# ZhonghuaYi/FocusFlow_official

Hardware: AMD Instinct MI355X
Metric: frame-pairs/sec FF-RAFT 384x512 iters=12 (higher is better)
Workload: dtype f32 via fp16x3 split operands on the f16 MFMA pipe (f32 accumulate, fp32-level accuracy); 1 GPU; FF-RAFT forward (test_mode), 8 pairs/GPU 384x512, iters=12, fp32 correlation pyramid, random-init weights, ORB-like masks (BASELINE configs[1]); pairs_per_gpu=8, corr_pyramid=fp32, conv_precision=f16x3, hipgraph=False, skip_unused_upsample=False, parallelism=dp1 (independent shards, no collective)

## Files before the change

### focusflow_official_amd/_hip.py

```python
import ctypes as C
import os

_PKG = os.path.dirname(os.path.abspath(__file__))
LIB_PATH = os.path.join(_PKG, "lib", "libfocusflow_hip.so")
if os.environ.get("FF_LAB_LIB"):
    LIB_PATH = os.path.join(_PKG, "lib", os.environ["FF_LAB_LIB"])

ACT_NONE, ACT_RELU, ACT_SIGMOID, ACT_TANH, ACT_LEAKY = 0, 1, 2, 3, 4
W_F32, W_F16X3, W_F16 = 0, 1, 2
MAX_SEG = 3
_fp = C.c_void_p
_ll = C.c_longlong


class FFFusionPair(C.Structure):
    _fields_ = [
        ("x", _fp * 2), ("x_ld", C.c_int * 2), ("xres", _fp * 2), ("xres_ld", C.c_int * 2), ("scale", _fp * 2), ("shift", _fp * 2),
        ("in_act", C.c_int), ("w_frag", _fp * 2), ("bias", _fp * 2), ("w_format", C.c_int), ("y", _fp * 2), ("y_ld", C.c_int * 2),
        ("B", C.c_int), ("HW", C.c_int), ("C", C.c_int),
    ]


class FFConvParams(C.Structure):
    _fields_ = [
# ... 17 lines not shown

PACK_MAX_MEMBERS = 4
PACK_MAX_SLICES = 4


class FFPackJob(C.Structure):
    _fields_ = [
        ("w", _fp * PACK_MAX_MEMBERS), ("bias", _fp * PACK_MAX_MEMBERS),
        ("cout_m", C.c_int * PACK_MAX_MEMBERS), ("off", C.c_int * PACK_MAX_MEMBERS), ("nmem", C.c_int), ("cout", C.c_int),
        ("cin_src", C.c_int), ("nslice", C.c_int), ("slice_lo", C.c_int * PACK_MAX_SLICES), ("slice_hi", C.c_int * PACK_MAX_SLICES),
        ("cin", C.c_int), ("cin_pad", C.c_int), ("KH", C.c_int), ("KW", C.c_int),
        ("fwd", _fp), ("bias_dst", _fp), ("dgrad", _fp),
        ("fwd_format", C.c_int), ("dgrad_format", C.c_int), ("cout_pad", C.c_int), ("reserved", C.c_int),
        ("items_fwd", _ll), ("items_dgrad", _ll), ("block0", _ll),
    ]


_SIGS = {
    "ff_pack_job_check": [C.POINTER(FFPackJob)],
    "ff_pack_weights_table": [_fp, C.c_int, _ll, _fp],
    "ff_unpack_wgrad_group": [_fp, _fp, C.c_int, C.POINTER(C.c_int), C.POINTER(C.c_int), C.POINTER(C.c_int), C.c_int, C.c_int,
                              C.POINTER(C.c_int), C.POINTER(C.c_int), C.c_int, C.c_int, C.c_int, _fp, _fp],
    "ff_conv2d_fwd": [C.POINTER(FFConvParams), _fp],
    "ff_pack_conv_weight": [_fp, C.c_int, C.c_int, C.c_int, C.c_int, _fp, C.c_int, C.c_int, _fp],
    "ff_pack_split_f16": [_fp, _fp, _ll, C.c_int, _fp],
    "ff_pack_frag16": [_fp, _fp, C.c_int, C.c_int, _fp],
    "ff_norm_stats": [_fp, C.c_int, C.c_int, C.c_int, C.c_int, C.c_int, _fp, _fp],
    "ff_norm_stats_finish": [_fp, C.c_int, C.c_int, C.c_int, _fp, _fp],
    "ff_mask_upsample_pack": [_fp, _fp, _fp],
    "ff_mask_upsample_fwd": [_fp, C.c_int, _fp, C.c_int, _fp, C.c_float, _fp, C.c_int, _fp, C.c_int, C.c_int, C.c_int, _fp],
    "ff_probe_memory_kernel": [_fp, _ll, _fp, _ll, C.c_int, C.c_int, C.c_int, C.c_uint, C.POINTER(C.c_longlong), C.POINTER(C.c_longlong), _fp],
    "ff_launch_timing_begin": [C.c_int],
    "ff_launch_timing_end": [C.c_int, C.POINTER(C.c_longlong), C.POINTER(C.c_double), C.POINTER(C.c_double), C.POINTER(C.c_double)],
    "ff_norm_apply": [_fp, C.c_int, _fp, C.c_int, C.c_int, C.c_int, C.c_int, _fp, C.c_int, C.c_float,
                      _fp, _fp, C.c_int, _fp, C.c_int, _fp],
    "ff_norm_coeffs": [_fp, C.c_int, C.c_int, _ll, C.c_float, _fp, _fp, _fp, _fp, _fp],
    "ff_bn_fold": [_fp, _fp, _fp, _fp, C.c_float, _fp, _fp, C.c_int, _fp],
    "ff_bn_update_running": [_fp, _ll, C.c_float, _fp, _fp, C.c_int, _fp],
    "ff_prep_input": [_fp, C.c_int, C.c_float, _fp, C.c_int, C.c_int, C.c_int, _fp],
    "ff_corr_pyramid": [_fp, _fp, _fp, _fp, _ll, C.c_int, C.c_int, _fp],
    "ff_corr_lookup_fwd": [C.POINTER(_fp), C.c_int, C.c_int, _fp, _ll, C.c_int, C.c_int, _fp, C.c_int, _fp, _fp],
    "ff_corr_build": [_fp, _fp, C.POINTER(_fp), C.c_int, C.c_int, C.c_int, C.c_int, C.c_int, _fp],
    "ff_corr_retile": [_fp, _fp, _ll, C.c_int, C.c_int, C.c_int, C.c_int, C.c_int, _fp],
    "ff_corr_tile_rows": [_fp, _fp, C.c_int, C.c_int, C.c_int, C.c_int, C.c_int, _fp],
    "ff_corr_lookup_tiled_fwd": [C.POINTER(_fp), C.c_int, _fp, _ll, C.c_int, C.c_int, _fp, C.c_int, _fp, _fp],
    "ff_corr_lookup_tiled_bwd_all": [_fp, C.POINTER(_fp), C.POINTER(_fp), C.c_int, C.c_int, _ll, C.c_int, C.c_int, _fp],
# ... 147 lines not shown
```

### focusflow_official_amd/csrc/conv_patch.hip

```cpp
#include <algorithm>
#include <cstdlib>
#include "ff_common.h"

namespace {

typedef float f32x16 __attribute__((ext_vector_type(16)));
typedef float f32x4 __attribute__((ext_vector_type(4)));
typedef _Float16 f16x8 __attribute__((ext_vector_type(8)));
typedef _Float16 f16x4 __attribute__((ext_vector_type(4)));

constexpr int TW = 16, ROWB = 128;
constexpr int ROWP = 144;
__device__ __forceinline__ int PI16(int i) { return (i >= 4 && i < 12) ? 2 * (i - 4) : (i < 4 ? 2 * i + 1 : 2 * (i - 12) + 9); }
__device__ __forceinline__ int KG16(int g) { return ((g & 1) << 1) | (g >> 1); }


struct PArgs {
    FFConvParams p;
    int Cin, nci;
    int tiles_x, tiles_y, n_tiles;
    long long w_row_bytes;
    int nci_split;
};

__device__ __forceinline__ void split4(const f32x4 v, f16x4& h0, f16x4& h1) {
#pragma unroll
    for (int j = 0; j < 4; ++j) {
        const _Float16 a = (_Float16)v[j];
        h0[j] = a;
        h1[j] = (_Float16)(v[j] - (float)a);
    }
}

template <int TERMS, int NITEM, int TM, int TN, int ABL, int WB, bool PIN = false, bool INORM = false, bool SPLITK = false, bool MF16 = false, int EPI = 0, bool STATS = false>
__device__ __forceinline__ void conv_patch_body(const PArgs& a) {
    constexpr int TH = 4 * TM, BN = 64 * TN, NW = 2 * TN;
    extern __shared__ __attribute__((aligned(16))) char smem[];
    const FFConvParams& p = a.p;
    float xs, xinv;
    ff::input_scale(p.x_amax, xs, xinv);
    xs *= ff::XSPLIT; xinv *= ff::SPLIT_INV;
    const int KH = p.KH, KW = p.KW, PH = TH + KH - 1, PW = TW + KW - 1, NPIX = PH * PW;
    char* sP = smem;
    char* sW = smem + ((NPIX * ROWP + 255) & ~255);

// ... 262 lines not shown

    const int li = lane & 31, lh = lane >> 5;
    const int rot = (KW - 1) & 15;
    const int lrow = li >> 4, lcol = ((li & 15) - lrow * rot) & 15;
    const int ntaps = KH * KW;
    const int brow = wn * TN * 32 + li;
    const char* abase[TM];
#pragma unroll
    for (int t = 0; t < TM; ++t) abase[t] = sP + (((wm * TM + t) * 2 + lrow) * PW + lcol) * ROWP + lh * 16;

    f16x8 abl_f;
#pragma unroll
    for (int i = 0; i < 8; ++i) abl_f[i] = (_Float16)(0.37f + 0.01f * (float)((lane * 7 + i * 3) & 31));
    const int c_beg = SPLITK ? (int)blockIdx.y * a.nci_split : 0;
    const int c_end = SPLITK ? min(c_beg + a.nci_split, a.nci) : a.nci;
    load_patch(c_beg);
    load_w(c_beg);
    int wbuf = 0;
    for (int c = c_beg; c < c_end; ++c) {
        __syncthreads();
        if (ABL != 6 || c == c_beg) store_patch();
        store_w(wbuf);
        __syncthreads();
        if (c + 1 < c_end && ABL != 6) load_patch(c + 1);
        for (int tap = 0; tap < ntaps; ++tap) {
            const bool last = tap + 1 == ntaps;
            const int next_kc = last ? (c + 1) : (tap + 1) * a.nci + c;
            if (!(last && c + 1 == c_end) && ABL != 1 && ABL != 2) load_w(last ? c + 1 : next_kc);
            if (PIN) __builtin_amdgcn_sched_barrier(0);
            const int dy = tap / KW, dx = tap - dy * KW;
            const int tapoff = (dy * PW + dx) * ROWP;
            const char* cW = sW + wbuf * BN * ROWP + brow * ROWP + lh * 16;
#pragma unroll
            for (int s = 0; s < 2; ++s) {
                f16x8 a0[TM], a1[TM], b0[TN], b1[TN];
                if constexpr (ABL == 5) {
#pragma unroll
                    for (int t = 0; t < TM; ++t) { a0[t] = abl_f; a1[t] = abl_f; }
#pragma unroll
                    for (int j = 0; j < TN; ++j) { b0[j] = abl_f; b1[j] = abl_f; }
                    asm volatile("" : "+v"(abl_f));
                } else {
#pragma unroll
                for (int t = 0; t < TM; ++t) {
                    const char* pa = abase[t] + tapoff;
                    a0[t] = *reinterpret_cast<const f16x8*>(pa + s * 32);
                    if (TERMS == 3) a1[t] = *reinterpret_cast<const f16x8*>(pa + 64 + s * 32);
// ... 3 lines not shown
                    b0[j] = *reinterpret_cast<const f16x8*>(cW + j * 32 * ROWP + s * 32);
                    if (TERMS == 3) b1[j] = *reinterpret_cast<const f16x8*>(cW + j * 32 * ROWP + 64 + s * 32);
                }
                }
#pragma unroll
                for (int t = 0; t < TM; ++t)
#pragma unroll
                    for (int j = 0; j < TN; ++j) {
                        if constexpr (ABL == 3) {
                            asm volatile("" :: "v"(a0[t]), "v"(b0[j]));
                            if (TERMS == 3) asm volatile("" :: "v"(a1[t]), "v"(b1[j]));
                            continue;
                        }
                        acc[t][j] = __builtin_amdgcn_mfma_f32_32x32x16_f16(a0[t], b0[j], acc[t][j], 0, 0, 0);
                        if (TERMS == 3) {
                            acc[t][j] = __builtin_amdgcn_mfma_f32_32x32x16_f16(a0[t], b1[j], acc[t][j], 0, 0, 0);
                            acc[t][j] = __builtin_amdgcn_mfma_f32_32x32x16_f16(a1[t], b0[j], acc[t][j], 0, 0, 0);
                        }
                    }
            }
            if (!last && ABL != 2) {
                if (WB == 1 && ABL != 4) __syncthreads();
                store_w(WB == 1 ? 0 : wbuf ^ 1);
                if (ABL != 4) __syncthreads();
                if (WB == 2) wbuf ^= 1;
            }
        }
        if (WB == 2) wbuf ^= 1;
    }

    if constexpr (SPLITK) {
        float* ws = p.splitk_ws + (long long)blockIdx.y * pix_total * p.Cout;
#pragma unroll
        for (int j = 0; j < TN; ++j) {
            const int n = n0 + (wn * TN + j) * 32 + li;
            if (n >= p.Cout) continue;
#pragma unroll
            for (int t = 0; t < TM; ++t)
#pragma unroll
                for (int r = 0; r < 16; ++r) {
                    const int pi = (r & 3) + 8 * (r >> 2) + 4 * lh;
                    const int y = y0 + (wm * TM + t) * 2 + (pi >> 4), x = x0 + ((pi - (pi >> 4) * rot) & 15);
                    if (y < H && x < W) ws[(((long long)bimg * H + y) * W + x) * p.Cout + n] = acc[t][j][r] * xinv;
                }
        }
        return;
// ... 77 lines not shown
}

template <int TERMS, int NITEM, int TM, int TN, int ABL = 0, int WB = 2>
__global__ __launch_bounds__(256) void conv_patch_kernel(const PArgs a) { conv_patch_body<TERMS, NITEM, TM, TN, ABL, WB>(a); }
template <int TERMS, int NITEM, int TM, int TN, int OCC, bool PIN = true, int ABL = 0, bool INORM = false, bool SPLITK = false, bool MF16 = false, int EPI = 0, bool STATS = false>
__global__ __launch_bounds__(256) __attribute__((amdgpu_waves_per_eu(OCC, OCC))) void conv_patch_kernel_occ(const PArgs a) { conv_patch_body<TERMS, NITEM, TM, TN, ABL, 1, PIN, INORM, SPLITK, MF16, EPI, STATS>(a); }

__global__ __launch_bounds__(256) void splitk_finish_kernel(const FFConvParams p, int splits, long long npix) {
    const long long total = npix * p.Cout;
    for (long long i = blockIdx.x * 256ll + threadIdx.x; i < total; i += (long long)gridDim.x * 256) {
        const long long m = i / p.Cout;
        const int n = (int)(i - m * p.Cout);
        float v = 0.f;
        for (int s = 0; s < splits; ++s) v += p.splitk_ws[(long long)s * total + i];
        v += p.bias ? p.bias[n] : 0.f;
        v *= p.out_scale;
        if (p.ch_scale) v = v * p.ch_scale[n] + p.ch_shift[n];
        v = ff::apply_act(v, p.act);
        if (p.res) v = ff::apply_act(v + p.res[m * p.res_ld + n], p.act_res);
        p.y[m * p.y_ld + n] = v;
    }
}

template <int TERMS, int NITEM, int TM, int TN, int OCC>
int launch_occ(const PArgs& a, size_t lds, hipStream_t s) {
    const long long blocks = (long long)a.p.B * a.tiles_y * a.tiles_x * a.n_tiles;
    static const bool mf16 = ff::tune_env("FF_MFMA16") && atoi(ff::tune_env("FF_MFMA16")) == 1;
    if (a.p.stats_part) {
        if (a.p.in_scale) conv_patch_kernel_occ<TERMS, NITEM, TM, TN, OCC, true, 0, true, false, false, 0, true><<<(unsigned)blocks, 256, lds, s>>>(a);
        else conv_patch_kernel_occ<TERMS, NITEM, TM, TN, OCC, true, 0, false, false, false, 0, true><<<(unsigned)blocks, 256, lds, s>>>(a);
        return ff::check_launch("ff_conv2d_fwd(patch, statistics)");
    }
    if (a.p.ep_mode) {
        if (a.p.ep_mode == FF_EP_GRU_RH) conv_patch_kernel_occ<TERMS, NITEM, TM, TN, OCC, true, 0, false, false, true, FF_EP_GRU_RH><<<(unsigned)blocks, 256, lds, s>>>(a);
        else conv_patch_kernel_occ<TERMS, NITEM, TM, TN, OCC, true, 0, false, false, true, FF_EP_GRU_BLEND><<<(unsigned)blocks, 256, lds, s>>>(a);
        return ff::check_launch("ff_conv2d_fwd(patch, GRU epilogue)");
    }
    if (mf16) {
        if (a.p.splitk > 1) {
            const int splits = (a.nci + a.nci_split - 1) / a.nci_split;
            conv_patch_kernel_occ<TERMS, NITEM, TM, TN, OCC, true, 0, false, true, true><<<dim3((unsigned)blocks, splits), 256, lds, s>>>(a);
            const long long npix = (long long)a.p.B * a.p.H * a.p.W, total = npix * a.p.Cout;
            splitk_finish_kernel<<<(unsigned)std::min<long long>((total + 255) / 256, 2048), 256, 0, s>>>(a.p, splits, npix);
            return ff::check_launch("ff_conv2d_fwd(patch, split-K)");
        }
        if (a.p.in_scale) conv_patch_kernel_occ<TERMS, NITEM, TM, TN, OCC, true, 0, true, false, true><<<(unsigned)blocks, 256, lds, s>>>(a);
        else conv_patch_kernel_occ<TERMS, NITEM, TM, TN, OCC, true, 0, false, false, true><<<(unsigned)blocks, 256, lds, s>>>(a);
        return ff::check_launch("ff_conv2d_fwd(patch)");
    }
    if (a.p.splitk > 1) {
        const int splits = (a.nci + a.nci_split - 1) / a.nci_split;
        conv_patch_kernel_occ<TERMS, NITEM, TM, TN, OCC, true, 0, false, true><<<dim3((unsigned)blocks, splits), 256, lds, s>>>(a);
        const long long npix = (long long)a.p.B * a.p.H * a.p.W, total = npix * a.p.Cout;
        splitk_finish_kernel<<<(unsigned)std::min<long long>((total + 255) / 256, 2048), 256, 0, s>>>(a.p, splits, npix);
        return ff::check_launch("ff_conv2d_fwd(patch, split-K)");
    }
    static const bool pin = !(ff::tune_env("FF_PATCH_PIN") && atoi(ff::tune_env("FF_PATCH_PIN")) == 0);
    if (a.p.in_scale) {
        conv_patch_kernel_occ<TERMS, NITEM, TM, TN, OCC, true, 0, true><<<(unsigned)blocks, 256, lds, s>>>(a);
        return ff::check_launch("ff_conv2d_fwd(patch)");
    }
#ifdef FF_LAB
    static const int oabl = getenv("FF_PATCH_ABLATE") ? atoi(getenv("FF_PATCH_ABLATE")) : 0;
#define FF_OCC_ABL(ENV_, ABL_) \
    if (oabl == ENV_) { conv_patch_kernel_occ<TERMS, NITEM, TM, TN, OCC, true, ABL_><<<(unsigned)blocks, 256, lds, s>>>(a); return ff::check_launch("ff_conv2d_fwd(patch)"); }
    FF_OCC_ABL(4, 4) FF_OCC_ABL(11, 1) FF_OCC_ABL(12, 2) FF_OCC_ABL(13, 3) FF_OCC_ABL(15, 5) FF_OCC_ABL(16, 6)
#undef FF_OCC_ABL
#endif
    if (!pin) {
        conv_patch_kernel_occ<TERMS, NITEM, TM, TN, OCC, false><<<(unsigned)blocks, 256, lds, s>>>(a);
        return ff::check_launch("ff_conv2d_fwd(patch)");
    }
    conv_patch_kernel_occ<TERMS, NITEM, TM, TN, OCC><<<(unsigned)blocks, 256, lds, s>>>(a);
    return ff::check_launch("ff_conv2d_fwd(patch)");
}

template <int NITEM, int TM, int TN, int OCC>
int launch_occ_f16(const PArgs& a, size_t lds, hipStream_t s) {
    const long long blocks = (long long)a.p.B * a.tiles_y * a.tiles_x * a.n_tiles;
    if (a.p.stats_part) {
        if (a.p.in_scale) conv_patch_kernel_occ<1, NITEM, TM, TN, OCC, true, 0, true, false, false, 0, true><<<(unsigned)blocks, 256, lds, s>>>(a);
        else conv_patch_kernel_occ<1, NITEM, TM, TN, OCC, true, 0, false, false, false, 0, true><<<(unsigned)blocks, 256, lds, s>>>(a);
        return ff::check_launch("ff_conv2d_fwd(patch, f16, statistics)");
    }
    if (a.p.ep_mode) {
        if (a.p.ep_mode == FF_EP_GRU_RH) conv_patch_kernel_occ<1, NITEM, TM, TN, OCC, true, 0, false, false, true, FF_EP_GRU_RH><<<(unsigned)blocks, 256, lds, s>>>(a);
        else conv_patch_kernel_occ<1, NITEM, TM, TN, OCC, true, 0, false, false, true, FF_EP_GRU_BLEND><<<(unsigned)blocks, 256, lds, s>>>(a);
        return ff::check_launch("ff_conv2d_fwd(patch, f16, GRU epilogue)");
    }
// ... 1 lines not shown
        const int splits = (a.nci + a.nci_split - 1) / a.nci_split;
        conv_patch_kernel_occ<1, NITEM, TM, TN, OCC, true, 0, false, true><<<dim3((unsigned)blocks, splits), 256, lds, s>>>(a);
        const long long npix = (long long)a.p.B * a.p.H * a.p.W, total = npix * a.p.Cout;
        splitk_finish_kernel<<<(unsigned)std::min<long long>((total + 255) / 256, 2048), 256, 0, s>>>(a.p, splits, npix);
        return ff::check_launch("ff_conv2d_fwd(patch, f16, split-K)");
    }
    if (a.p.in_scale) conv_patch_kernel_occ<1, NITEM, TM, TN, OCC, true, 0, true><<<(unsigned)blocks, 256, lds, s>>>(a);
    else conv_patch_kernel_occ<1, NITEM, TM, TN, OCC><<<(unsigned)blocks, 256, lds, s>>>(a);
    return ff::check_launch("ff_conv2d_fwd(patch, f16)");
}

template <int TERMS, int NITEM, int TM, int TN, int ABL = 0, int WB = 2>
int launch(const PArgs& a, size_t lds, hipStream_t s) {
    static bool once = false;
    if (!once) {
        (void)hipFuncSetAttribute(reinterpret_cast<const void*>(&conv_patch_kernel<TERMS, NITEM, TM, TN, ABL, WB>), hipFuncAttributeMaxDynamicSharedMemorySize, 96 * 1024);
        once = true;
    }
    const long long blocks = (long long)a.p.B * a.tiles_y * a.tiles_x * a.n_tiles;
    conv_patch_kernel<TERMS, NITEM, TM, TN, ABL, WB><<<(unsigned)blocks, 256, lds, s>>>(a);
    return ff::check_launch("ff_conv2d_fwd(patch)");
}

}

namespace ff {
int conv2d_fwd_patch(const FFConvParams& p, int cin, hipStream_t s) {
    static const bool enabled = !ff::tune_env("FF_NO_PATCH_CONV");
    static const bool dbg = ff::tune_env("FF_DEBUG_DISPATCH") != nullptr;
    if (dbg) fprintf(stderr, "[ff] patch? en=%d stride=%d dil=%d,%d groups=%d k=%dx%d pad=%d,%d cin=%d xc=%d,%d,%d fmt=%d\n", (int)enabled, p.stride,
                     p.dil_h, p.dil_w, p.groups, p.KH, p.KW, p.pad_h, p.pad_w, cin, p.x_c[0], p.x_c[1], p.x_c[2], p.w_format);
    if (!enabled) return 1;
    const int dlh = p.dil_h ? p.dil_h : 1, dlw = p.dil_w ? p.dil_w : 1;
    if (p.stride != 1 || dlh != 1 || dlw != 1 || p.groups != 1) return 1;
    if (p.KH % 2 == 0 || p.KW % 2 == 0 || p.pad_h != p.KH / 2 || p.pad_w != p.KW / 2 || p.KH > 7 || p.KW > 7) return 1;
    if (p.KH * p.KW < 3) return 1;
    if (cin % 32) return 1;
    long long max_bytes = 0;
    for (int i = 0; i < FF_MAX_SEG; ++i) {
        if (p.x_c[i] % 32) return 1;
        if (p.x_c[i]) max_bytes = std::max(max_bytes, (long long)p.B * p.H * p.W * p.x_ld[i] * 4);
    }
    PArgs a;
    a.p = p;
    a.Cin = cin;
    a.nci = cin / 32;
    a.tiles_x = (p.W + TW - 1) / TW;
    a.w_row_bytes = (long long)((p.KH * p.KW * cin + 31) / 32) * ROWB;
    max_bytes = std::max(max_bytes, (long long)p.Cout * a.w_row_bytes);
    if (max_bytes >= (1ll << 31)) return 1;
    static const int force_th = ff::tune_env("FF_PATCH_TH") ? atoi(ff::tune_env("FF_PATCH_TH")) : 0;
    static const int force_tn = ff::tune_env("FF_PATCH_TN") ? atoi(ff::tune_env("FF_PATCH_TN")) : 0;
    auto nblocks = [&](int th, int tn) { return (long long)p.B * ((p.H + th - 1) / th) * a.tiles_x * ((p.Cout + 64 * tn - 1) / (64 * tn)); };
    int th = nblocks(8, 1) < 512 ? 4 : 8, tn = 1;
    if (force_th) th = force_th;
    if (force_tn) tn = force_tn;
    a.tiles_y = (p.H + th - 1) / th;
    a.n_tiles = (p.Cout + 64 * tn - 1) / (64 * tn);
    const int npix = (th + p.KH - 1) * (TW + p.KW - 1);
    static const int lds_pad = ff::tune_env("FF_PATCH_LDS_PAD") ? atoi(ff::tune_env("FF_PATCH_LDS_PAD")) : 0;
    const int nitem = (npix * 8 + 255) / 256;
    const bool t3 = p.w_format == FF_W_F16X3;
    static const int wb1 = ff::tune_env("FF_PATCH_WB1") ? atoi(ff::tune_env("FF_PATCH_WB1")) : 3;
    const bool occ = (t3 || p.w_format == FF_W_F16) && tn == 1 && ((th == 8 && nitem <= 6 && (wb1 & 1)) || (th == 4 && nitem <= 4 && (wb1 & 2)));
    const size_t lds = ((npix * ROWP + 255) & ~255) + (occ ? 1 : 2) * 64 * tn * ROWP + lds_pad;
    if (lds > 96 * 1024) return 1;
#ifdef FF_LAB
    static const int abl = getenv("FF_PATCH_ABLATE") ? atoi(getenv("FF_PATCH_ABLATE")) : 0;
    if (abl >= 1 && abl <= 3 && th == 8 && tn == 1 && nitem <= 6 && t3) {
        if (abl == 1) return launch<3, 6, 2, 1, 1>(a, lds, s);
        if (abl == 2) return launch<3, 6, 2, 1, 2>(a, lds, s);
        return launch<3, 6, 2, 1, 3>(a, lds, s);
    }
#endif
    if (p.y_fmt != FF_FMT_F32) {
        static const bool mf16 = ff::tune_env("FF_MFMA16") && atoi(ff::tune_env("FF_MFMA16")) == 1;
        if (!occ || p.ep_mode || p.splitk > 1 || mf16) return 1;
    }
    if (!(occ && th == 4 && p.splitk > 1 && p.splitk_ws && !p.in_scale && !p.res2)) a.p.splitk = 0;
    a.nci_split = a.p.splitk > 1 ? (a.nci + a.p.splitk - 1) / a.p.splitk : a.nci;
    if (p.stats_part && (!occ || a.p.splitk > 1 || p.ep_mode))
        return ff::fail(FF_EINVAL, "ff_conv2d_fwd: stats_part: ask ff_conv2d_stats_parts first (this convolution cannot produce statistics)");
    if (p.ep_mode) {
        if (!occ || a.p.splitk > 1 || p.in_scale || p.Cout % 4) return ff::fail(FF_EINVAL, "ff_conv2d_fwd: ep_mode needs the f16x3 patch kernel's 8x16 / 4x16 tiles (got %dx%d kernel, Cin %d, Cout %d)", p.KH, p.KW, cin, p.Cout);
    }
    if (occ && !t3) return th == 8 ? launch_occ_f16<6, 2, 1, 4>(a, lds, s) : launch_occ_f16<4, 1, 1, 5>(a, lds, s);
    if (occ) return th == 8 ? launch_occ<3, 6, 2, 1, 4>(a, lds, s) : launch_occ<3, 4, 1, 1, 5>(a, lds, s);
    if (p.in_scale) return 1;
#define FF_PATCH_CASE(TH_, TN_, NI_) \
    if (th == TH_ && tn == TN_ && nitem <= NI_) return t3 ? launch<3, NI_, TH_ / 4, TN_>(a, lds, s) : launch<1, NI_, TH_ / 4, TN_>(a, lds, s);
    FF_PATCH_CASE(8, 1, 6) FF_PATCH_CASE(8, 1, 10)
    FF_PATCH_CASE(4, 1, 4) FF_PATCH_CASE(4, 1, 8)
    FF_PATCH_CASE(8, 2, 6) FF_PATCH_CASE(8, 2, 10)
    FF_PATCH_CASE(4, 2, 4) FF_PATCH_CASE(4, 2, 8)
    FF_PATCH_CASE(16, 1, 11) FF_PATCH_CASE(16, 1, 16)
#undef FF_PATCH_CASE
    return 1;
}

int conv2d_stats_parts(const FFConvParams& p, int cin) {
    static const bool enabled = !ff::tune_env("FF_NO_PATCH_CONV") && !(getenv("FF_CONV_STATS") && atoi(getenv("FF_CONV_STATS")) == 0);
    if (!enabled || (p.w_format != FF_W_F16X3 && p.w_format != FF_W_F16) || p.res2 || p.ep_mode || p.x_amax) return 0;
    const int dlh = p.dil_h ? p.dil_h : 1, dlw = p.dil_w ? p.dil_w : 1;
    if (p.stride != 1 || dlh != 1 || dlw != 1 || p.groups != 1) return 0;
    if (p.KH % 2 == 0 || p.KW % 2 == 0 || p.pad_h != p.KH / 2 || p.pad_w != p.KW / 2 || p.KH > 7 || p.KW > 7 || p.KH * p.KW < 3) return 0;
    if (cin % 32) return 0;
    for (int i = 0; i < FF_MAX_SEG; ++i)
        if (p.x_c[i] % 32) return 0;
    if (ff::tune_env("FF_PATCH_TH") || ff::tune_env("FF_PATCH_TN") || ff::tune_env("FF_PATCH_WB1")) return 0;
    long long max_bytes = (long long)p.Cout * ((p.KH * p.KW * cin + 31) / 32) * ROWB;
    for (int i = 0; i < FF_MAX_SEG; ++i)
        if (p.x_c[i]) max_bytes = std::max(max_bytes, (long long)p.B * p.H * p.W * p.x_ld[i] * 4);
    if (max_bytes >= (1ll << 31)) return 0;
    const int tiles_x = (p.W + TW - 1) / TW, n_tiles = (p.Cout + 63) / 64;
    const int th = (long long)p.B * ((p.H + 7) / 8) * tiles_x * n_tiles < 512 ? 4 : 8;
    const int npix = (th + p.KH - 1) * (TW + p.KW - 1), nitem = (npix * 8 + 255) / 256;
    if (!((th == 8 && nitem <= 6) || (th == 4 && nitem <= 4))) return 0;
    if (th == 4 && p.splitk > 1 && p.splitk_ws) return 0;
    return ((p.H + th - 1) / th) * tiles_x * 2;
}

int conv2d_splitk_hint(const FFConvParams& p, int cin) {
    static const bool enabled = !ff::tune_env("FF_NO_PATCH_CONV") && !(ff::tune_env("FF_SPLITK") && atoi(ff::tune_env("FF_SPLITK")) == 0);
    if (!enabled || p.w_format != FF_W_F16X3 || p.in_scale || p.res2) return 0;
    const int dlh = p.dil_h ? p.dil_h : 1, dlw = p.dil_w ? p.dil_w : 1;
    if (p.stride != 1 || dlh != 1 || dlw != 1 || p.groups != 1) return 0;
    if (p.KH % 2 == 0 || p.KW % 2 == 0 || p.pad_h != p.KH / 2 || p.pad_w != p.KW / 2 || p.KH * p.KW < 3) return 0;
    if (cin % 32) return 0;
    for (int i = 0; i < FF_MAX_SEG; ++i)
        if (p.x_c[i] % 32) return 0;
    const int tiles_x = (p.W + TW - 1) / TW, n_tiles = (p.Cout + 63) / 64;
    if ((long long)p.B * ((p.H + 7) / 8) * tiles_x * n_tiles >= 512) return 0;
    const int npix = (4 + p.KH - 1) * (TW + p.KW - 1);
    if ((npix * 8 + 255) / 256 > 4) return 0;
    const long long blocks = (long long)p.B * ((p.H + 3) / 4) * tiles_x * n_tiles;
    const int nci = cin / 32;
    if (blocks > 256 || nci < 6 || nci * p.KH * p.KW <= (p.splitk < 0 ? 36 : 72)) return 0;
    const int splits = (int)std::min<long long>(std::min(16, nci / 2), 768 / blocks);
// ... 4 lines not shown
```

### focusflow_official_amd/ops.py

```python
import ctypes as C
import math
import os
import threading
from typing import List, Optional, Sequence

import torch

from . import _hip
from ._hip import ACT_LEAKY, ACT_NONE, ACT_RELU, ACT_SIGMOID, ACT_TANH, FFConvParams

Tensor = torch.Tensor


_raw_stream = getattr(torch._C, "_cuda_getCurrentRawStream", None)
_raw_device = getattr(torch._C, "_cuda_getDevice", None)


def _stream():
    if _raw_stream is not None and _raw_device is not None:
        return C.c_void_p(_raw_stream(_raw_device()))
    return C.c_void_p(torch.cuda.current_stream().cuda_stream)


_PRECISIONS = {"fp32": _hip.W_F32, "f16x3": _hip.W_F16X3, "f16": _hip.W_F16}
# ... 14 lines not shown
def w_format() -> int:
    return _PRECISIONS[_conv_precision]


def pack_split(rows_f32: Tensor) -> Tensor:
    _require_gpu(rows_f32)
    rows, k = rows_f32.shape
    assert rows_f32.is_contiguous()
    dst = torch.empty((rows, (k + 31) // 32 * 128), dtype=torch.uint8, device=rows_f32.device)
    _hip.call("ff_pack_split_f16", _p(rows_f32), _p(dst), rows, k, _stream())
    return dst


def pack_frag16(w_split: Tensor, rows: int) -> Tensor:
    nkc = w_split.shape[1] // 128
    dst = torch.empty(((rows + 15) // 16) * nkc * 2048, dtype=torch.uint8, device=w_split.device)
    _hip.call("ff_pack_frag16", _p(w_split), _p(dst), rows, nkc, _stream())
    return dst


class _StreamPolicy(threading.local):
    single_stream = False
    encoder_streams_ok = True


policy = _StreamPolicy()

_prof_on = False
_prof_events = {}
_prof_notes = {}


def profile_begin(*labels: str):
    global _prof_on
    _prof_on = True
    _prof_events.clear()
    _prof_notes.clear()
    for lb in labels:
        _prof_events[lb] = []
        _prof_notes[lb] = []


def profile_end():
    global _prof_on
    _prof_on = False
    torch.cuda.synchronize()
# ... 101 lines not shown

def split_copy(x: Tensor, act: int = ACT_NONE, to_split: bool = True, out: Optional[Tensor] = None):
    b, h, w, c = x.shape
    if out is None:
        out = empty_nhwc(b, h, w, c, x)
    _hip.call("ff_split_copy", _p(x), _ld(x), _p(out), _ld(out), b * h * w, c, act, 1 if to_split else 0, _stream())
    return SplitT(out) if to_split else out


def pack_conv_weight(w_oihw: Tensor, dst: Tensor, cin_pad: int, cout_offset: int = 0):
    _require_gpu(w_oihw)
    co, ci, kh, kw = w_oihw.shape
    assert dst.is_contiguous() and dst.shape[1] == kh * kw * cin_pad and dst.shape[0] >= cout_offset + co
    _hip.call("ff_pack_conv_weight", _p(w_oihw.contiguous()), co, ci, kh, kw, _p(dst), cin_pad, cout_offset, _stream())


def conv2d(xs: Sequence[Tensor], wpack: Tensor, bias: Optional[Tensor], cout: int, kh: int, kw: int,
           stride: int = 1, pad=(0, 0), act: int = ACT_NONE, out: Optional[Tensor] = None,
           res: Optional[Tensor] = None, act_res: int = ACT_NONE, ch_scale: Optional[Tensor] = None,
           ch_shift: Optional[Tensor] = None, out_scale: float = 1.0, w_fmt: int = 0, dilation: int = 1,
           x_amax: Optional[Tensor] = None, in_scale: Optional[Tensor] = None, in_shift: Optional[Tensor] = None,
           in_act: int = ACT_NONE, res2: Optional[Tensor] = None, res_split: int = 0,
           ep_rh: Optional[Tensor] = None, ep_split: int = 0, ep_blend=None, want_stats: bool = False, ep_coords=None,
           y_split=False, y2_split: bool = False, ep_motion_tail: Optional[Tensor] = None, w_frag: Optional[Tensor] = None):
    if isinstance(pad, int):
        pad = (pad, pad)
    fmts = [1 if isinstance(x, SplitT) else 0 for x in xs]
    xs = [_raw(x) for x in xs]
    x0 = xs[0]
    b, h, w, _ = x0.shape
    ho = (h + 2 * pad[0] - dilation * (kh - 1) - 1) // stride + 1
    wo = (w + 2 * pad[1] - dilation * (kw - 1) - 1) // stride + 1
    if out is None:
        if y_split is not False:
            full = empty_nhwc(b, ho, wo, (cout + 31) // 32 * 32, x0)
            out = full if full.shape[3] == cout else full[..., :cout]
        else:
            out = empty_nhwc(b, ho, wo, (cout + 3) // 4 * 4, x0)[..., :cout] if cout % 4 else empty_nhwc(b, ho, wo, cout, x0)
    p = FFConvParams()
    cin = 0
    for i, x in enumerate(xs):
        assert x.shape[:3] == x0.shape[:3]
        p.x[i] = x.data_ptr()
        p.x_ld[i] = _ld(x)
        p.x_c[i] = x.shape[3]
        p.x_gstride[i] = 0
        p.x_fmt[i] = fmts[i]
# ... 43 lines not shown
    assert out.shape[:3] == (b, ho, wo) and out.shape[3] >= cout
    if _range_word is not None and w_fmt and x_amax is None and in_scale is None:
        for x, f in zip(xs, fmts):
            if not f:
                _range_probe(x)
    klen = cin * kh * kw
    plain = not any(fmts) and y_split is False and not y2_split
    if plain and w_fmt and not p.ep_mode and b * ho * wo <= 16384 and klen > 1152:
        short = klen <= 2304
        if not short or torch.cuda.is_current_stream_capturing():
            p.splitk = -1 if short else 0
            nsplit = _hip.load().ff_conv2d_splitk_hint(C.byref(p))
            p.splitk = 0
            if nsplit > 1:
                ws = torch.empty(nsplit * b * ho * wo * cout, dtype=torch.float32, device=x0.device)
                p.splitk_ws, p.splitk = ws.data_ptr(), nsplit
    nparts = _hip.load().ff_conv2d_stats_parts(C.byref(p)) if want_stats and CONV_STATS and not p.splitk else 0
    if nparts:
        parts = torch.empty(b * nparts * cout * 4, dtype=torch.float32, device=x0.device)
        p.stats_part = parts.data_ptr()
        _timed_call("conv", "ff_conv2d_fwd", C.byref(p), _stream(), note=(2.0 * b * ho * wo * cout * kh * kw * cin, w_fmt))
        stats = _zero_stats(b, cout, x0.device)
        _hip.call("ff_norm_stats_finish", _p(parts), b, nparts, cout, _p(stats), _stream())
        return out, stats
    _timed_call("conv", "ff_conv2d_fwd", C.byref(p), _stream(), note=(2.0 * b * ho * wo * cout * kh * kw * cin, w_fmt))
    if want_stats:
        return out, norm_stats(out, per_sample=True)
    if y_split is True:
        out = SplitT(out)
    if y2_split:
        return out, SplitT(out2)
    return out


class TiledPyramid:

    def __init__(self, levels: List[Tensor], h0: int, w0: int, half: bool):
        self.levels, self.h0, self.w0, self.half = levels, h0, w0, half

    @staticmethod
    def plane_elems(h0: int, w0: int, level: int, half: bool) -> int:
        n = _hip.load().ff_corr_plane_elems(h0, w0, level, int(half))
        if n <= 0:
            raise _hip.FocusFlowHipError(f"ff_corr_plane_elems({h0}, {w0}, {level}) failed")
        return n

# ... 1117 lines not shown
```

### include/focusflow_hip.h

```cpp
#ifndef FOCUSFLOW_HIP_H
#define FOCUSFLOW_HIP_H

#ifdef __cplusplus
extern "C" {
#endif

#define FF_OK 0
#define FF_EINVAL (-1)
#define FF_EHIP (-2)

#define FF_ACT_NONE 0
#define FF_ACT_RELU 1
#define FF_ACT_SIGMOID 2
#define FF_ACT_TANH 3
#define FF_ACT_LEAKY 4

#define FF_MAX_SEG 3

#define FF_W_F32 0
#define FF_W_F16X3 1
#define FF_W_F16 2

const char* ff_last_error(void);
#define FF_ABI_VERSION 7
// ... 54 lines not shown
    int x_fmt[FF_MAX_SEG];
    int y_fmt;
    int y_fmt_from;
    float* y2;
    int y2_ld;
    const void* w_frag;
} FFConvParams;
#define FF_FMT_F32 0
#define FF_FMT_SPLIT 1
#define FF_EP_NONE 0
#define FF_EP_GRU_RH 1
#define FF_EP_GRU_BLEND 2
#define FF_EP_COORDS 3
#define FF_EP_MOTION_TAIL 4

int ff_conv2d_fwd(const FFConvParams* p, void* stream);

int ff_pack_conv_weight(const float* w_oihw, int Cout, int Cin, int KH, int KW,
                        float* dst, int cin_pad, int cout_offset, void* stream);
int ff_pack_split_f16(const float* src_rows, void* dst, long long rows, int K, void* stream);
int ff_pack_frag16(const void* split_rows, void* dst, int rows, int nkc, void* stream);
int ff_conv2d_splitk_hint(const FFConvParams* p);
int ff_conv2d_stats_parts(const FFConvParams* p);

int ff_norm_stats(const float* x, int ld, int B, int HW, int C, int per_sample,
                  double* stats, void* stream);
int ff_norm_stats_finish(const float* parts, int B, int nparts, int C, double* stats, void* stream);
int ff_norm_apply(const float* x, int ld, float* y, int y_ld, int B, int HW, int C,
                  const double* stats, int per_sample, float eps,
                  const float* gamma, const float* beta, int act,
                  const float* res, int res_ld, void* stream);
int ff_norm_coeffs(const double* stats, int S, int C, long long count, float eps, const float* gamma, const float* beta,
                   float* scale, float* shift, void* stream);
int ff_bn_fold(const float* running_mean, const float* running_var, const float* gamma,
               const float* beta, float eps, float* ch_scale, float* ch_shift, int C, void* stream);
int ff_bn_update_running(const double* stats, long long count, float momentum,
                         float* running_mean, float* running_var, int C, void* stream);

int ff_prep_input(const float* src_nchw, int src_c, float fill_value, float* dst_nhwc4,
                  int B, int H, int W, void* stream);

int ff_corr_pyramid(const float* lvl0, float* lvl1, float* lvl2, float* lvl3,
                    long long planes, int h0, int w0, void* stream);
int ff_corr_lookup_fwd(const float* const* levels ,
                       int num_levels, int radius, const float* coords ,
                       long long queries, int h0, int w0, float* out, int out_ld,
// ... 206 lines not shown
```

Baseline: 627.5 frame-pairs/s.

## Add warp-specialized loader-role conv kernel processing multiple x-tiles per block

Adds a new 3x3 patch conv kernel where one wave loads weights and three waves load and convert the input patch, and each block walks a run of x-tiles while prefetching the next tile's first channel chunk. An auto route picks it for f16x3 residual or stats convs with Cin 64/96 when there are enough blocks. The aim is to overlap global loads with MFMA work and amortise the patch prologue across tiles. In exchange it adds fixed waves-per-EU occupancy and extra barriers, and the new path is chosen automatically by shape heuristics. An extra ablation mode also moves the next-patch prefetch into the tap loop.

```diff
diff --git a/focusflow_official_amd/_hip.py b/focusflow_official_amd/_hip.py
--- a/focusflow_official_amd/_hip.py
+++ b/focusflow_official_amd/_hip.py
@@ -63,6 +63,7 @@
     "ff_unpack_wgrad_group": [_fp, _fp, C.c_int, C.POINTER(C.c_int), C.POINTER(C.c_int), C.POINTER(C.c_int), C.c_int, C.c_int,
                               C.POINTER(C.c_int), C.POINTER(C.c_int), C.c_int, C.c_int, C.c_int, _fp, _fp],
     "ff_conv2d_fwd": [C.POINTER(FFConvParams), _fp],
+    "ff_conv_patch_route": [C.c_int],
     "ff_pack_conv_weight": [_fp, C.c_int, C.c_int, C.c_int, C.c_int, _fp, C.c_int, C.c_int, _fp],
     "ff_pack_split_f16": [_fp, _fp, _ll, C.c_int, _fp],
     "ff_pack_frag16": [_fp, _fp, C.c_int, C.c_int, _fp],
diff --git a/focusflow_official_amd/csrc/conv_patch.hip b/focusflow_official_amd/csrc/conv_patch.hip
--- a/focusflow_official_amd/csrc/conv_patch.hip
+++ b/focusflow_official_amd/csrc/conv_patch.hip
@@ -21,6 +21,7 @@
     int tiles_x, tiles_y, n_tiles;
     long long w_row_bytes;
     int nci_split;
+    int tile_run, tiles_xg;
 };
 
 __device__ __forceinline__ void split4(const f32x4 v, f16x4& h0, f16x4& h1) {
@@ -329,7 +330,7 @@
         if (ABL != 6 || c == c_beg) store_patch();
         store_w(wbuf);
         __syncthreads();
-        if (c + 1 < c_end && ABL != 6) load_patch(c + 1);
+        if (c + 1 < c_end && ABL != 6 && ABL != 7) load_patch(c + 1);
         for (int tap = 0; tap < ntaps; ++tap) {
             const bool last = tap + 1 == ntaps;
             const int next_kc = last ? (c + 1) : (tap + 1) * a.nci + c;
@@ -379,6 +380,7 @@
             if (!last && ABL != 2) {
                 if (WB == 1 && ABL != 4) __syncthreads();
                 store_w(WB == 1 ? 0 : wbuf ^ 1);
+                if (ABL == 7 && tap == 0 && c + 1 < c_end) load_patch(c + 1);
                 if (ABL != 4) __syncthreads();
                 if (WB == 2) wbuf ^= 1;
             }
@@ -502,6 +504,262 @@
     }
 }
 
+template <int TERMS, bool INORM, bool STATS>
+__global__ __launch_bounds__(256) __attribute__((amdgpu_waves_per_eu(4, 4))) void conv_patch_roles_kernel(const PArgs a) {
+    constexpr int KH = 3, KW = 3, TM = 2, TH = 4 * TM, PW = TW + KW - 1, NPIX = (TH + KH - 1) * PW, NS = 8;
+    constexpr int ROT = (KW - 1) & 15, OOB = 0x7fffffff;
+    static_assert(NS * 192 >= NPIX * 8, "patch items of the three loader waves");
+    extern __shared__ __attribute__((aligned(16))) char smem[];
+    const FFConvParams& p = a.p;
+    float xs, xinv;
+    ff::input_scale(p.x_amax, xs, xinv);
+    xs *= ff::XSPLIT; xinv *= ff::SPLIT_INV;
+    char* sP = smem;
+    char* sW = smem + ((NPIX * ROWP + 255) & ~255);
+
+    const int tid = threadIdx.x, lane = tid & 63;
+    const int wave = __builtin_amdgcn_readfirstlane(tid >> 6);
+    const bool wrole = wave == 3;
+    const int wm = wave >> 1, wn = wave & 1;
+    const int H = p.H, W = p.W, nci = a.nci;
+    int bid = blockIdx.x;
+    const int nt = bid % a.n_tiles; bid /= a.n_tiles;
+    const int txg = bid % a.tiles_xg; bid /= a.tiles_xg;
+    const int ty = bid % a.tiles_y;
+    const int bimg = bid / a.tiles_y;
+    const int tx0 = txg * a.tile_run, ntile = min(a.tile_run, a.tiles_x - tx0);
+    const int y0 = ty * TH, n0 = nt * 64;
+
+    const long long pix_total = (long long)p.B * H * W;
+    const int ldb = p.x_ld[0] * 4;
+    __amdgpu_buffer_rsrc_t rsx = __builtin_amdgcn_make_buffer_rsrc(const_cast<float*>(p.x[0]), 0, (int)(pix_total * ldb), 0x00020000);
+    __amdgpu_buffer_rsrc_t rsw = __builtin_amdgcn_make_buffer_rsrc(const_cast<float*>(p.w), 0, (int)((long long)p.Cout * a.w_row_bytes), 0x00020000);
+    __amdgpu_buffer_rsrc_t rsy = __builtin_amdgcn_make_buffer_rsrc(p.y, 0, (int)(pix_total * p.y_ld * 4), 0x00020000);
+    __amdgpu_buffer_rsrc_t rsr = __builtin_amdgcn_make_buffer_rsrc(const_cast<float*>(p.res ? p.res : p.y), 0, p.res ? (int)(pix_total * p.res_ld * 4) : 0, 0x00020000);
+
+    const int kq = tid & 7;
+    f32x4 st[NS];
+    f32x4 nmul = {1.f, 1.f, 1.f, 1.f}, nadd = {0.f, 0.f, 0.f, 0.f};
+    int inside = 0;
+    auto load_patch = [&](int c, int x0) {
+        if (INORM) {
+            const long long t = (long long)bimg * a.Cin + c * 32 + kq * 4;
+            nmul = *reinterpret_cast<const f32x4*>(p.in_scale + t);
+            nadd = *reinterpret_cast<const f32x4*>(p.in_shift + t);
+        }
+        int q = tid >> 3;
+        asm volatile("" : "+v"(q));
+        inside = 0;
+#pragma unroll
+        for (int i = 0; i < NS; ++i) {
+            const int px = q + 24 * i;
+            const int yy = y0 - KH / 2 + px / PW, xx = x0 - KW / 2 + px % PW;
+            const bool in = px < NPIX && (unsigned)yy < (unsigned)H && (unsigned)xx < (unsigned)W;
+            if (INORM) inside |= in ? 1 << i : 0;
+            st[i] = __builtin_bit_cast(f32x4, __builtin_amdgcn_raw_buffer_load_b128(rsx, in ? ((bimg * H + yy) * W + xx) * ldb + kq * 16 + c * 128 : OOB, 0, 0));
+        }
+    };
+    auto store_patch = [&]() {
+        const int pc = kq >> 1, half = (kq & 1) * 8;
+#pragma unroll
+        for (int i = 0; i < NS; ++i) {
+            const int row = (tid >> 3) + 24 * i;
+            if (row < NPIX) {
+                f16x4 h0, h1;
+                f32x4 v = st[i];
+                if (INORM) {
+                    v = __builtin_elementwise_fma(v, nmul, nadd);
+                    if (p.in_act == FF_ACT_RELU) {
+#pragma unroll
+                        for (int j = 0; j < 4; ++j) v[j] = v[j] < 0.f ? 0.f : v[j];
+                    }
+                    if (!(inside >> i & 1)) v = (f32x4){0.f, 0.f, 0.f, 0.f};
+                }
+                split4(v * xs, h0, h1);
+                *reinterpret_cast<f16x4*>(sP + row * ROWP + pc * 16 + half) = h0;
+                if (TERMS == 3) *reinterpret_cast<f16x4*>(sP + row * ROWP + 64 + pc * 16 + half) = h1;
+            }
+        }
+    };
+    const int wrow = n0 + (lane >> 3), woff = wrow * (int)a.w_row_bytes + kq * 16, wstep = 8 * (int)a.w_row_bytes;
+    auto load_w = [&](int kc) {
+#pragma unroll
+        for (int i = 0; i < NS; ++i)
+            st[i] = __builtin_bit_cast(f32x4, __builtin_amdgcn_raw_buffer_load_b128(rsw, wrow + 8 * i < p.Cout ? woff : OOB, kc * ROWB + i * wstep, 0));
+    };
+    auto store_w = [&]() {
+#pragma unroll
+        for (int i = 0; i < NS; ++i) *reinterpret_cast<f32x4*>(sW + ((lane >> 3) + 8 * i) * ROWP + kq * 16) = st[i];
+    };
+    auto stage = [&]() {
+        if (wrole) store_w();
+        else store_patch();
+    };
+
+    const int li = lane & 31, lh = lane >> 5;
+    const int lrow = li >> 4, lcol = ((li & 15) - lrow * ROT) & 15;
+    const char* abase[TM];
+#pragma unroll
+    for (int t = 0; t < TM; ++t) abase[t] = sP + (((wm * TM + t) * 2 + lrow) * PW + lcol) * ROWP + lh * 16;
+    const char* cW = sW + (wn * 32 + li) * ROWP + lh * 16;
+
+    const int n = n0 + wn * 32 + li, nc = min(n, p.Cout - 1);
+    const bool nok = n < p.Cout;
+    const float bias = p.bias ? p.bias[nc] : 0.f;
+    const float cs = p.ch_scale ? p.ch_scale[nc] : 1.f;
+    const float ct = p.ch_scale ? p.ch_shift[nc] : 0.f;
+    const int npix_all = (int)pix_total;
+    auto act8 = [&](float (&v)[8], int act) {
+#define FF_ACT8(CODE_)                                              \
+    case CODE_:                                                     \
+        _Pragma("unroll") for (int k = 0; k < 8; ++k) v[k] = ff::apply_act(v[k], CODE_); \
+        break;
+        switch (act) {
+            FF_ACT8(FF_ACT_RELU) FF_ACT8(FF_ACT_SIGMOID) FF_ACT8(FF_ACT_TANH) FF_ACT8(FF_ACT_LEAKY)
+            default: break;
+        }
+#undef FF_ACT8
+    };
+
+    if (wrole) load_w(0);
+    else load_patch(0, tx0 * TW);
+    stage();
+    for (int tl = 0; tl < ntile; ++tl) {
+        const int tx = tx0 + tl, x0 = tx * TW;
+        const bool more = tl + 1 < ntile;
+        f32x16 acc[TM];
+#pragma unroll
+        for (int t = 0; t < TM; ++t)
+#pragma unroll
+            for (int r = 0; r < 16; ++r) acc[t][r] = 0.f;
+        for (int c = 0; c < nci; ++c) {
+            const bool lastc = c + 1 == nci;
+            if (c > 0) {
+                __syncthreads();
+                stage();
+            }
+            __syncthreads();
+            if (!wrole) {
+                if (!lastc) load_patch(c + 1, x0);
+                else if (more) load_patch(0, x0 + TW);
+            }
+#pragma unroll
+            for (int tap = 0; tap < KH * KW; ++tap) {
+                constexpr int NTAP = KH * KW;
+                const bool last = tap + 1 == NTAP;
+                if (wrole && !(last && lastc && !more)) load_w(last ? (lastc ? 0 : c + 1) : (tap + 1) * nci + c);
+                __builtin_amdgcn_sched_barrier(0);
+                const int tapoff = ((tap / KW) * PW + tap % KW) * ROWP;
+#pragma unroll
+                for (int s = 0; s < 2; ++s) {
+                    f16x8 a0[TM], a1[TM], b0, b1;
+#pragma unroll
+                    for (int t = 0; t < TM; ++t) {
+                        const char* pa = abase[t] + tapoff;
+                        a0[t] = *reinterpret_cast<const f16x8*>(pa + s * 32);
+                        if (TERMS == 3) a1[t] = *reinterpret_cast<const f16x8*>(pa + 64 + s * 32);
+                    }
+                    b0 = *reinterpret_cast<const f16x8*>(cW + s * 32);
+                    if (TERMS == 3) b1 = *reinterpret_cast<const f16x8*>(cW + 64 + s * 32);
+#pragma unroll
+                    for (int t = 0; t < TM; ++t) {
+                        acc[t] = __builtin_amdgcn_mfma_f32_32x32x16_f16(a0[t], b0, acc[t], 0, 0, 0);
+                        if (TERMS == 3) {
+                            acc[t] = __builtin_amdgcn_mfma_f32_32x32x16_f16(a0[t], b1, acc[t], 0, 0, 0);
+                            acc[t] = __builtin_amdgcn_mfma_f32_32x32x16_f16(a1[t], b0, acc[t], 0, 0, 0);
+                        }
+                    }
+                }
+                if (!last) {
+                    __syncthreads();
+                    if (wrole) store_w();
+                    __syncthreads();
+                }
+            }
+        }
+        __syncthreads();
+        if (more) stage();
+
+        float st_p = 0.f, st_s1 = 0.f, st_s2 = 0.f, st_n = 0.f;
+#pragma unroll
+        for (int th = 0; th < 2 * TM; ++th) {
+            int lhq = lh;
+            asm volatile("" : "+v"(lhq));
+            const int t = th >> 1, r0 = (th & 1) * 8;
+            float vv[8];
+            int pixi[8];
+#pragma unroll
+            for (int k = 0; k < 8; ++k) {
+                const int r = r0 + k;
+                float v = acc[t][r] * xinv + bias;
+                v *= p.out_scale;
+                if (p.ch_scale) v = v * cs + ct;
+                vv[k] = v;
+                const int pi = (r & 3) + 8 * (r >> 2) + 4 * lhq;
+                const int y = y0 + (wm * TM + t) * 2 + (r >> 3), x = x0 + ((pi - (r >> 3) * ROT) & 15);
+                pixi[k] = (y < H && x < W && nok) ? (bimg * H + y) * W + x : npix_all;
+            }
+            act8(vv, p.act);
+            if (p.res) {
+                float rr[8];
+#pragma unroll
+                for (int k = 0; k < 8; ++k)
+                    rr[k] = __builtin_bit_cast(float, __builtin_amdgcn_raw_buffer_load_b32(rsr, (pixi[k] * p.res_ld + n) * 4, 0, 0));
+#pragma unroll
+                for (int k = 0; k < 8; ++k) vv[k] = vv[k] + rr[k];
+                act8(vv, p.act_res);
+            }
+#pragma unroll
+            for (int k = 0; k < 8; ++k)
+                __builtin_amdgcn_raw_buffer_store_b32(__builtin_bit_cast(unsigned int, vv[k]), rsy, (pixi[k] * p.y_ld + n) * 4, 0, 0);
+            if constexpr (STATS) {
+                if (y0 + TH <= H && x0 + TW <= W) {
+                    if (th == 0) st_p = vv[0];
+#pragma unroll
+                    for (int k = 0; k < 8; ++k) {
+                        const float d = vv[k] - st_p;
+                        st_s1 += d;
+                        st_s2 = fmaf(d, d, st_s2);
+                    }
+                    st_n += 8.f;
+                } else {
+#pragma unroll
+                    for (int k = 0; k < 8; ++k) {
+                        if (pixi[k] == npix_all) continue;
+                        if (st_n == 0.f) st_p = vv[k];
+                        const float d = vv[k] - st_p;
+                        st_s1 += d;
+                        st_s2 = fmaf(d, d, st_s2);
+                        st_n += 1.f;
+                    }
+                }
+            }
+        }
+        if constexpr (STATS) {
+            const float p2 = __shfl_xor(st_p, 32), s2 = __shfl_xor(st_s1, 32), q2 = __shfl_xor(st_s2, 32), n2 = __shfl_xor(st_n, 32);
+            if (lh == 0 && nok) {
+                const float pv = st_n > 0.f ? st_p : p2, d = p2 - pv;
+                const float s1 = st_s1 + s2 + n2 * d;
+                const float q1 = st_s2 + q2 + 2.f * d * s2 + n2 * d * d;
+                const int part = (ty * a.tiles_x + tx) * 2 + wm;
+                const int nparts = a.tiles_y * a.tiles_x * 2;
+                *reinterpret_cast<f32x4*>(p.stats_part + (((long long)bimg * nparts + part) * p.Cout + n) * 4) = (f32x4){pv, s1, q1, st_n + n2};
+            }
+        }
+    }
+}
+
+template <int TERMS>
+int launch_roles(const PArgs& a, size_t lds, hipStream_t s) {
+    const unsigned blocks = (unsigned)((long long)a.p.B * a.tiles_y * a.tiles_xg * a.n_tiles);
+    const bool norm = a.p.in_scale != nullptr, stats = a.p.stats_part != nullptr;
+    if (norm && stats) conv_patch_roles_kernel<TERMS, true, true><<<blocks, 256, lds, s>>>(a);
+    else if (norm) conv_patch_roles_kernel<TERMS, true, false><<<blocks, 256, lds, s>>>(a);
+    else if (stats) conv_patch_roles_kernel<TERMS, false, true><<<blocks, 256, lds, s>>>(a);
+    else conv_patch_roles_kernel<TERMS, false, false><<<blocks, 256, lds, s>>>(a);
+    return ff::check_launch("ff_conv2d_fwd(patch, loader roles)");
+}
+
 template <int TERMS, int NITEM, int TM, int TN, int OCC>
 int launch_occ(const PArgs& a, size_t lds, hipStream_t s) {
     const long long blocks = (long long)a.p.B * a.tiles_y * a.tiles_x * a.n_tiles;
@@ -544,7 +802,7 @@
     static const int oabl = getenv("FF_PATCH_ABLATE") ? atoi(getenv("FF_PATCH_ABLATE")) : 0;
 #define FF_OCC_ABL(ENV_, ABL_) \
     if (oabl == ENV_) { conv_patch_kernel_occ<TERMS, NITEM, TM, TN, OCC, true, ABL_><<<(unsigned)blocks, 256, lds, s>>>(a); return ff::check_launch("ff_conv2d_fwd(patch)"); }
-    FF_OCC_ABL(4, 4) FF_OCC_ABL(11, 1) FF_OCC_ABL(12, 2) FF_OCC_ABL(13, 3) FF_OCC_ABL(15, 5) FF_OCC_ABL(16, 6)
+    FF_OCC_ABL(4, 4) FF_OCC_ABL(11, 1) FF_OCC_ABL(12, 2) FF_OCC_ABL(13, 3) FF_OCC_ABL(15, 5) FF_OCC_ABL(16, 6) FF_OCC_ABL(17, 7)
 #undef FF_OCC_ABL
 #endif
     if (!pin) {
@@ -592,6 +850,29 @@
     return ff::check_launch("ff_conv2d_fwd(patch)");
 }
 
+thread_local int g_patch_route = 0;
+
+bool roles_shape(const FFConvParams& p, int cin) {
+    if (p.KH != 3 || p.KW != 3 || (cin != 64 && cin != 96) || p.x_c[0] != cin || p.x_fmt[0] != FF_FMT_F32) return false;
+    if (p.w_format != FF_W_F16X3 && p.w_format != FF_W_F16) return false;
+    if (p.y_fmt != FF_FMT_F32 || p.y2 || p.ep_mode || p.res2 || p.splitk > 1) return false;
+    const long long pix = (long long)p.B * p.H * p.W;
+    return pix * p.y_ld * 4 < (1ll << 31) && (!p.res || pix * p.res_ld * 4 < (1ll << 31));
+}
+
+int roles_auto_run(const FFConvParams& p, int cin) {
+    if (p.in_scale || p.w_format != FF_W_F16X3) return 0;
+    if (!(p.res || (p.stats_part && cin == 64))) return 0;
+    const long long blocks = (long long)p.B * ((p.H + 7) / 8) * ((((p.W + TW - 1) / TW) + 1) / 2) * ((p.Cout + 63) / 64);
+    return blocks >= 512 ? 2 : 0;
+}
+
+}
+
+extern "C" int ff_conv_patch_route(int mode) {
+    FF_REQUIRE(mode == 0 || mode == 1 || mode == 2 || mode == 4, "ff_conv_patch_route: mode %d (0 = by shape, 1 = shipped instance, 2 / 4 = loader roles, tiles per block)", mode);
+    g_patch_route = mode;
+    return FF_OK;
 }
 
 namespace ff {
@@ -625,6 +906,8 @@
     int th = nblocks(8, 1) < 512 ? 4 : 8, tn = 1;
     if (force_th) th = force_th;
     if (force_tn) tn = force_tn;
+    const bool roles_ok = roles_shape(p, cin);
+    if (roles_ok && g_patch_route) th = 8;
     a.tiles_y = (p.H + th - 1) / th;
     a.n_tiles = (p.Cout + 64 * tn - 1) / (64 * tn);
     const int npix = (th + p.KH - 1) * (TW + p.KW - 1);
@@ -654,6 +937,13 @@
     if (p.ep_mode) {
         if (!occ || a.p.splitk > 1 || p.in_scale || p.Cout % 4) return ff::fail(FF_EINVAL, "ff_conv2d_fwd: ep_mode needs the f16x3 patch kernel's 8x16 / 4x16 tiles (got %dx%d kernel, Cin %d, Cout %d)", p.KH, p.KW, cin, p.Cout);
     }
+    if (occ && th == 8 && roles_ok && g_patch_route != 1) {
+        a.tile_run = g_patch_route ? g_patch_route : roles_auto_run(p, cin);
+        if (a.tile_run) {
+            a.tiles_xg = (a.tiles_x + a.tile_run - 1) / a.tile_run;
+            return t3 ? launch_roles<3>(a, lds, s) : launch_roles<1>(a, lds, s);
+        }
+    }
     if (occ && !t3) return th == 8 ? launch_occ_f16<6, 2, 1, 4>(a, lds, s) : launch_occ_f16<4, 1, 1, 5>(a, lds, s);
     if (occ) return th == 8 ? launch_occ<3, 6, 2, 1, 4>(a, lds, s) : launch_occ<3, 4, 1, 1, 5>(a, lds, s);
     if (p.in_scale) return 1;
@@ -683,7 +973,8 @@
         if (p.x_c[i]) max_bytes = std::max(max_bytes, (long long)p.B * p.H * p.W * p.x_ld[i] * 4);
     if (max_bytes >= (1ll << 31)) return 0;
     const int tiles_x = (p.W + TW - 1) / TW, n_tiles = (p.Cout + 63) / 64;
-    const int th = (long long)p.B * ((p.H + 7) / 8) * tiles_x * n_tiles < 512 ? 4 : 8;
+    int th = (long long)p.B * ((p.H + 7) / 8) * tiles_x * n_tiles < 512 ? 4 : 8;
+    if (g_patch_route && roles_shape(p, cin)) th = 8;
     const int npix = (th + p.KH - 1) * (TW + p.KW - 1), nitem = (npix * 8 + 255) / 256;
     if (!((th == 8 && nitem <= 6) || (th == 4 && nitem <= 4))) return 0;
     if (th == 4 && p.splitk > 1 && p.splitk_ws) return 0;
diff --git a/focusflow_official_amd/ops.py b/focusflow_official_amd/ops.py
--- a/focusflow_official_amd/ops.py
+++ b/focusflow_official_amd/ops.py
@@ -60,6 +60,15 @@
 class _StreamPolicy(threading.local):
     single_stream = False
     encoder_streams_ok = True
+
+    @property
+    def patch_route(self):
+        return self.__dict__.get("_patch_route", 0)
+
+    @patch_route.setter
+    def patch_route(self, mode):
+        _hip.call("ff_conv_patch_route", int(mode))
+        self.__dict__["_patch_route"] = int(mode)
 
 
 policy = _StreamPolicy()
@@ -207,7 +216,8 @@
            x_amax: Optional[Tensor] = None, in_scale: Optional[Tensor] = None, in_shift: Optional[Tensor] = None,
            in_act: int = ACT_NONE, res2: Optional[Tensor] = None, res_split: int = 0,
            ep_rh: Optional[Tensor] = None, ep_split: int = 0, ep_blend=None, want_stats: bool = False, ep_coords=None,
-           y_split=False, y2_split: bool = False, ep_motion_tail: Optional[Tensor] = None, w_frag: Optional[Tensor] = None):
+           y_split=False, y2_split: bool = False, ep_motion_tail: Optional[Tensor] = None, w_frag: Optional[Tensor] = None,
+           stats_parts_out: Optional[list] = None):
     if isinstance(pad, int):
         pad = (pad, pad)
     fmts = [1 if isinstance(x, SplitT) else 0 for x in xs]
@@ -297,6 +307,8 @@
         _timed_call("conv", "ff_conv2d_fwd", C.byref(p), _stream(), note=(2.0 * b * ho * wo * cout * kh * kw * cin, w_fmt))
         stats = _zero_stats(b, cout, x0.device)
         _hip.call("ff_norm_stats_finish", _p(parts), b, nparts, cout, _p(stats), _stream())
+        if stats_parts_out is not None:
+            stats_parts_out.append(parts.view(b, nparts, cout, 4))
         return out, stats
     _timed_call("conv", "ff_conv2d_fwd", C.byref(p), _stream(), note=(2.0 * b * ho * wo * cout * kh * kw * cin, w_fmt))
     if want_stats:
diff --git a/include/focusflow_hip.h b/include/focusflow_hip.h
--- a/include/focusflow_hip.h
+++ b/include/focusflow_hip.h
@@ -100,6 +100,7 @@
 int ff_pack_frag16(const void* split_rows, void* dst, int rows, int nkc, void* stream);
 int ff_conv2d_splitk_hint(const FFConvParams* p);
 int ff_conv2d_stats_parts(const FFConvParams* p);
+int ff_conv_patch_route(int mode);
 
 int ff_norm_stats(const float* x, int ld, int B, int HW, int C, int per_sample,
                   double* stats, void* stream);
```

Result: no change. 631.0 frame-pairs/s, median of 6 (+0.6%).
